# Stan994265/mVIL-Fusion

Hardware: AMD Instinct MI355X
Metric: sliding-window solve iterations/sec (10 KF, 1k feat, 30k LiDAR pts) (higher is better)
Workload: dtype f64; 1 GPU; BASELINE.json configs[1]: K=10 keyframes, L=1000 landmarks, 3068 visual factors, 24000 plane + 6000 edge LiDAR points, 9 IMU, 3 ICP, 4 LPS, prior n=70 (vil_marginalize of the preceding synthetic window, on the GPU); termination=function_tolerance, parallelism=1 GPU, step=one full window solve, inputs resident in HBM

## Files before the change

mvil-fusion_amd/csrc/vil_step.hpp:

```cpp
#pragma once
#include <type_traits>

#include "vil_dev.hpp"
#include "vil_factors.hpp"
#include "vil_finish.hpp"

namespace vd {

#define STEP_NB 4
#define CH_SLOTS 7
#define PF_N ((55 * 256 + VIL_STEP_THREADS - 1) / VIL_STEP_THREADS)

struct StepShared {
    Ctl c;
    double red[64];
    unsigned char tI[256], tJ[256];
    double xs[320], dinv[320];
    double y[320];
    double sc[320], dcs[320], gr[320], gn[320];
    double gd[320];
    double rt[320];
    double x0[328];
    unsigned char cst[48];
    double hs[12];
// ... 822 lines not shown
                a0 = fma(wr[i], y0, a0); a1 = fma(wr[i + 1], y1, a1); a2 = fma(wr[i + 2], y2, a2); a3 = fma(wr[i + 3], y3, a3);
                c0 = fma(nn[i], y0, c0); c1 = fma(nn[i + 1], y1, c1); c2 = fma(nn[i + 2], y2, c2); c3 = fma(nn[i + 3], y3, c3);
            }
            asm volatile("s_waitcnt lgkmcnt(0)" ::: "memory");
            s.y[kb + tt] = (a0 + a1) + (a2 + a3);
            crit = (c0 + c1) + (c2 + c3);
        }
        lds_barrier();
        if (t >= 64) {
            const int lim = kb - 16;
            for (int w0 = (t & ~63) - 64; w0 < lim; w0 += NT - 64) {
                const int c = w0 + (t & 63), cc = min(c, lim - 1);
                const int base = tl_base(blk, cc >> 4) + (cc & 15);
                double v0 = 0.0, v1 = 0.0, v2 = 0.0, v3 = 0.0;
#pragma unroll
                for (int r = 0; r < 16; r += 4) {
                    v0 = fma(A[base + r * TILE_RS], s.y[kb + r], v0);
                    v1 = fma(A[base + (r + 1) * TILE_RS], s.y[kb + r + 1], v1);
                    v2 = fma(A[base + (r + 2) * TILE_RS], s.y[kb + r + 2], v2);
                    v3 = fma(A[base + (r + 3) * TILE_RS], s.y[kb + r + 3], v3);
                }
                double yn = s.y[cc] - ((v0 + v1) + (v2 + v3));
                asm volatile("" : "+v"(yn));
                if (c < lim) s.y[cc] = yn;
            }
        }
    }
    lds_barrier();
}

struct ChainSrcStep {
    const double* S; int D; const double* sc_; const double* dcs_; const double* gd_; const double* u_; double mu;
    __device__ __forceinline__ double u(int i) const { return u_[i]; }
    int NP;
    __device__ __forceinline__ double raw(int i, int j) const { return S[(size_t)i * D + j]; }
    __device__ __forceinline__ double diag(int k, int i, int j) const { return raw(NP + 9 * k + i, NP + 9 * k + j); }
    __device__ __forceinline__ double sub(int k, int kn, int q, int c) const { return raw(NP + 9 * kn + q, NP + 9 * k + c); }
    __device__ __forceinline__ double prow(int r, int k, int c) const { return raw(r, NP + 9 * k + c); }
    __device__ __forceinline__ double sc(int j) const { return sc_[j]; }
    __device__ __forceinline__ double madd(int j) const { const double d = dcs_[j]; return mu * d * d; }
    __device__ __forceinline__ double rowscale(int r) const { return sc_[r]; }
    __device__ __forceinline__ double rhsraw(int j) const { return gd_[j]; }
    __device__ __forceinline__ void row_done(int, int r, double zr, double& q) const { q += 2.0 * u_[r] * zr; }
    __device__ __forceinline__ void wput(double* p, double v) const { *p = v; }
};

template <bool WLDS, class PUB, class SIDE>
__device__ __forceinline__ bool solve_chain(const DevP& P, const SysBuf& sb, StepShared& s, double* lds, const double mu, const bool cam, double& qpart, PUB pub, SIDE side) {
    const int t = vil_tid();
#ifdef VIL_STAMPS
    #define SSTAMP(k) do { if (t == 0) { long long tt_; asm volatile("s_memtime %0\n s_waitcnt lgkmcnt(0)" : "=s"(tt_) :: "memory"); P.dbg[40 + k] = tt_; } } while (0)
#else
    #define SSTAMP(k) do {} while (0)
#endif
    SSTAMP(0);
    const int K = P.K, D = P.D, NP = P.NV, R = NP + 1, T = (R + 15) >> 4, ntile = (T * (T + 1)) >> 1;
    const int RS = P.chain_rs, NB = 9 * K, m = K >> 1;
    double* Tl = lds;
    double* Wt = WLDS ? lds + ntile * TILE_SZ : P.M;
    const ChainLds L = chain_lds(lds + ntile * TILE_SZ + (WLDS ? (size_t)chain_wcols(K) * RS : 0), K);
    if (t < 8) chain_flag_set(L.flag + t, 0);
    __syncthreads();
    SSTAMP(1);
    if (t < 384) {
        const ChainSrcStep src{sb.S, D, s.sc, s.dcs, s.gd, s.y, mu, NP};
        double qc = 0.0;
        if (cam) chain_eliminate<true>(src, K, NP, RS, Wt, L, qc, P.dbg); else chain_eliminate<false>(src, K, NP, RS, Wt, L, qc, P.dbg);
        qpart += qc;
    } else {
        const int pl = t - 384, NE = ntile << 8;
        for (int e0 = pl; e0 < NE; e0 += 4 * 128) {
            double v[4]; int ii[4], jj[4];
#pragma unroll
            for (int u = 0; u < 4; ++u) {
                const int e = min(e0 + 128 * u, NE - 1), tile = e >> 8, w = e & 255;
                ii[u] = (s.tI[tile] << 4) + (w >> 4); jj[u] = (s.tJ[tile] << 4) + (w & 15);
                v[u] = sb.S[(size_t)min(ii[u], NP - 1) * D + min(jj[u], NP - 1)];
            }
#pragma unroll
            for (int u = 0; u < 4; ++u) {
                const int e = e0 + 128 * u;
                if (e >= NE) break;
                const int i = ii[u], j = jj[u];
                double mv = 0.0;
                if (i < NP && j <= i) {
                    if (cam) qpart += (i == j ? 1.0 : 2.0) * s.y[i] * v[u] * s.y[j];
                    mv = s.sc[i] * v[u] * s.sc[j];
                    if (i == j) mv += mu * s.dcs[i] * s.dcs[i];
                } else if (i == NP && j < NP) mv = s.sc[j] * s.gd[j];
                Tl[tl_phys(e)] = mv;
            }
        }
#ifdef VIL_STAMPS
        if (t == 384) { long long tt_; asm volatile("s_memtime %0\n s_waitcnt lgkmcnt(0)" : "=s"(tt_) :: "memory"); P.dbg[57] = tt_; P.dbg[58] = tt_; }
#endif
    }
    __syncthreads();
    SSTAMP(2);
    if (chain_flag_get(L.flag + 5)) return false;
    SSTAMP(3);
    auto schur = [&](d4* Creg, const int* tIJ) {
        const int lane = t & 63, row = lane & 15, kq = lane >> 4;
        if (P.skip_mask & 128) return;
        const int RS4 = 4 * RS;
#pragma unroll
        for (int u = 0; u < CH_SLOTS; ++u) {
            if (tIJ[u] < 0) continue;
            const int I = tIJ[u] >> 8, J = tIJ[u] & 255;
            const bool va = (I << 4) + row < R, vb = (J << 4) + row < R;
            const double* pa = Wt + kq * RS + (I << 4) + row;
            const double* pb = Wt + kq * RS + (J << 4) + row;
            d4 c4 = Creg[u];
            for (int kk = 0; kk < NB; kk += 32) {
                const double* qa = pa + kk * RS; const double* qb = pb + kk * RS;
                double av[8], bv[8];
#pragma unroll
                for (int g = 0; g < 8; ++g) { av[g] = qa[g * RS4]; bv[g] = qb[g * RS4]; }
#pragma unroll
                for (int g = 0; g < 8; ++g) {
                    const bool kv = kk + 4 * g + kq < NB;
                    c4 = __builtin_amdgcn_mfma_f64_16x16x4f64((va && kv) ? -av[g] : 0.0, (vb && kv) ? bv[g] : 0.0, c4, 0, 0, 0);
                }
            }
            Creg[u] = c4;
        }
    };
    if (!chol_lookahead<CH_SLOTS, false>(Tl, NP, s, schur)) return false;
    SSTAMP(4);
    back_subst(Tl, NP, s);
    pub();
    SSTAMP(5);
    double* tB = L.tB;
    {
        const int G = (4 * NB <= VIL_STEP_THREADS) ? 4 : 2;
        const int j = t / G, part = t - j * G;
        const int jc = min(j, NB - 1);
        double acc = 0.0;
        for (int rr = part; rr < NP; rr += G) acc += Wt[(size_t)jc * RS + rr] * s.y[rr];
        acc += __shfl_xor(acc, 1, 64);
        if (G == 4) acc += __shfl_xor(acc, 2, 64);
        if (j < NB && part == 0) tB[j] = Wt[(size_t)j * RS + NP] - acc;
    }
    __syncthreads();
    if (t < 64) chain_block_back(L.Ldg + 54 * m, nullptr, tB + 9 * m, nullptr, s.y + NP + 9 * m);
    __syncthreads();
    if (t < 64) { for (int k = m - 1; k >= 0; --k) chain_block_back(L.Ldg + 54 * k, L.Lsb + 82 * k, tB + 9 * k, s.y + NP + 9 * (k + 1), s.y + NP + 9 * k); }
    else if (t < 128) { for (int k = m + 1; k < K; ++k) chain_block_back(L.Ldg + 54 * k, L.Lsb + 82 * k, tB + 9 * k, s.y + NP + 9 * (k - 1), s.y + NP + 9 * k); }
    else if (t >= VIL_STEP_THREADS - 64) side();
    __syncthreads();
    SSTAMP(6);
    return true;
}

template <bool RW , class PUB, class SIDE>
__device__ __forceinline__ bool solve_prechain(const DevP& P, const SysBuf& sb, StepShared& s, double* lds, const double mu, const bool cam, double& qpart, const int epoch , PUB pub, SIDE side) {
    const int t = vil_tid();
    SSTAMP(0);
    const int K = P.K, D = P.D, NP = P.NV, R = NP + 1, T = (R + 15) >> 4, ntile = (T * (T + 1)) >> 1;
    const int RS = P.chain_rs, NB = 9 * K, m = K >> 1;
    double* Tl = lds;
    const double* Wt = P.chW;
    double* Ldg = lds + ntile * TILE_SZ; double* Lsb = Ldg + 54 * K; double* tB = Lsb + 82 * K;
    {
        const int NE = ntile << 8;
        for (int e0 = t; e0 < NE; e0 += 8 * VIL_STEP_THREADS) {
            double v[8]; int ii[8], jj[8];
#pragma unroll
            for (int u = 0; u < 8; ++u) {
                const int e = min(e0 + VIL_STEP_THREADS * u, NE - 1), tile = e >> 8, w = e & 255;
                ii[u] = (s.tI[tile] << 4) + (w >> 4); jj[u] = (s.tJ[tile] << 4) + (w & 15);
                v[u] = ld_ag(sb.S + (size_t)min(ii[u], NP - 1) * D + min(jj[u], NP - 1));
            }
#pragma unroll
            for (int u = 0; u < 8; ++u) {
                const int e = e0 + VIL_STEP_THREADS * u;
                if (e >= NE) break;
                const int i = ii[u], j = jj[u];
                double mv = 0.0;
                if (i < NP && j <= i) {
                    if (cam) qpart += (i == j ? 1.0 : 2.0) * s.y[i] * v[u] * s.y[j];
                    mv = s.sc[i] * v[u] * s.sc[j];
                    if (i == j) mv += mu * s.dcs[i] * s.dcs[i];
                } else if (i == NP && j < NP) mv = s.sc[j] * s.gd[j];
                Tl[tl_phys(e)] = mv;
            }
        }
    }
    if (P.rs_merged) {
        for (int i = t; i < P.n_ww; i += VIL_STEP_THREADS) spin_until_eq(P.wwflag + i, epoch, P.abortf);
        __syncthreads();
    }
    if (t == 0) prof_stamp(P, epoch - 1, 9);
    SSTAMP(1);
    const int f2 = (P.rs_merged || P.prechain == 2) ? ld_ag(P.chflag + 2) : 0;
    {
        const int NE = ntile << 8;
        for (int e0 = t; e0 < NE; e0 += 8 * VIL_STEP_THREADS) {
            double ww[8];
#pragma unroll
            for (int u = 0; u < 8; ++u) ww[u] = ld_ag(P.chWW + tl_phys(min(e0 + VIL_STEP_THREADS * u, NE - 1)));
#pragma unroll
            for (int u = 0; u < 8; ++u) {
                const int e = e0 + VIL_STEP_THREADS * u;
                if (e >= NE) break;
                const int tile = e >> 8, w = e & 255, i = (s.tI[tile] << 4) + (w >> 4), j = (s.tJ[tile] << 4) + (w & 15);
                if (i <= NP && j <= i && j < NP) Tl[tl_phys(e)] -= (i < NP ? s.sc[i] : 1.0) * ww[u] * s.sc[j];
            }
        }
        if (cam) {
            if (t < NP) qpart += 2.0 * s.y[t] * (ld_ag(P.chZ + t) + ld_ag(P.chZ + R + t));
            if (t == 0) qpart += ld_ag(P.chQ) + ld_ag(P.chQ + 1);
        }
        if (t == 0 && !ld_ag(P.chOk)) s.ok = 0;
    }
    __syncthreads();
    SSTAMP(2); SSTAMP(3);
    if (!s.ok) return false;
    const int G = (4 * NB <= VIL_STEP_THREADS) ? 4 : 2;
    const int j = t / G, part = t - j * G;
    const int jc = min(j, NB - 1);
    double wv[24], wrhs = 0.0;
    const bool small = ntile <= 24;
    if (small) {
        const bool wave_has_columns = __builtin_amdgcn_readfirstlane(((t >> 6) << 6) / G) < NB;
#pragma unroll
        for (int q = 0; q < 24; ++q) wv[q] = 0.0;
        if (wave_has_columns) {
#pragma unroll
            for (int q = 0; q < 24; ++q) wv[q] = ld_ag(Wt + (size_t)jc * RS + min(part + q * G, NP - 1));
            wrhs = ld_ag(Wt + (size_t)jc * RS + NP);
        }
        if (!(RW ? chol_dense<3>(Tl, NP, s) : chol_lookahead<3, false>(Tl, NP, s))) return false;
    } else if (!(RW ? chol_dense<CH_SLOTS>(Tl, NP, s) : chol_lookahead<CH_SLOTS, false>(Tl, NP, s))) return false;
    SSTAMP(4);
    if (t == 0) prof_stamp(P, epoch - 1, 10);
    if (RW) back_subst_cols(Tl, NP, s); else back_subst(Tl, NP, s);
    pub();
    if (t == 0) prof_stamp(P, epoch - 1, 11);
    SSTAMP(5);
    {
        if (P.rs_merged || P.prechain == 2) {
            if (f2 != epoch) spin_until_eq(P.chflag + 2, epoch, P.abortf);
        }
        double acc = 0.0, pl[2], ps[2];
        const int nr = (NP - part + G - 1) / G;
#pragma unroll
        for (int q = 0; q < 2; ++q) { pl[q] = ld_ag(P.chLdg + min(t + q * VIL_STEP_THREADS, 54 * K - 1)); ps[q] = ld_ag(P.chLsb + min(t + q * VIL_STEP_THREADS, 82 * K - 1)); }
#pragma unroll
        for (int q = 0; q < 2; ++q) { const int e = t + q * VIL_STEP_THREADS; if (e < 54 * K) Ldg[e] = pl[q]; if (e < 82 * K) Lsb[e] = ps[q]; }
        for (int e = t + 2 * VIL_STEP_THREADS; e < 54 * K; e += VIL_STEP_THREADS) Ldg[e] = ld_ag(P.chLdg + e);
        for (int e = t + 2 * VIL_STEP_THREADS; e < 82 * K; e += VIL_STEP_THREADS) Lsb[e] = ld_ag(P.chLsb + e);
        if (small) {
#pragma unroll
            for (int q = 0; q < 24; ++q) { const int rr = min(part + q * G, NP - 1); acc += (q < nr ? wv[q] : 0.0) * s.sc[rr] * s.y[rr]; }
            for (int q = 24; q < nr; ++q) { const int rr = part + q * G; acc += ld_ag(Wt + (size_t)jc * RS + rr) * s.sc[rr] * s.y[rr]; }
            acc += __shfl_xor(acc, 1, 64);
            if (G == 4) acc += __shfl_xor(acc, 2, 64);
            if (j < NB && part == 0) tB[j] = wrhs - acc;
        } else {
            const int wave = t >> 6, lane = t & 63;
            const int r0 = min(lane, NP - 1), r1 = min(lane + 64, NP - 1);
            const double x0 = lane < NP ? s.sc[r0] * s.y[r0] : 0.0, x1 = lane + 64 < NP ? s.sc[r1] * s.y[r1] : 0.0;
            for (int j0 = wave; j0 < NB; j0 += 64) {
                double w0[8], w1[8], wr[8];
#pragma unroll
                for (int u = 0; u < 8; ++u) {
                    const double* col = Wt + (size_t)min(j0 + 8 * u, NB - 1) * RS;
                    w0[u] = ld_ag(col + r0); w1[u] = ld_ag(col + r1); wr[u] = ld_ag(col + NP);
                }
#pragma unroll
                for (int u = 0; u < 8; ++u) {
                    const double a = wave_total(w0[u] * x0 + w1[u] * x1);
                    if (lane == 0 && j0 + 8 * u < NB) tB[j0 + 8 * u] = wr[u] - a;
                }
            }
        }
    }
    __syncthreads();
    if (t < NB) {
        const int k = t / 9, r = t - 9 * k;
        const double* Li = Ldg + 54 * k; const double* tk = tB + 9 * k;
        double a0 = 0.0, a1 = 0.0;
#pragma unroll
        for (int i = 0; i < 9; ++i) { const double li = i >= r ? Li[(i * (i + 1) >> 1) + r] : 0.0; if (i & 1) a1 += li * tk[i]; else a0 += li * tk[i]; }
        s.y[NP + t] = a0 + a1;
    }
    __syncthreads();
    if (t < 128) {
        const int dir = t >> 6, lane = t & 63, r = min(lane, 8), stp = dir == 0 ? -1 : 1, kend = dir == 0 ? -1 : K;
        double xn = s.y[NP + 9 * m + r];
        int k = m + stp;
        double mrow[9], c = 0.0;
        auto fetch = [&](int kk, double* mr, double& cc) {
            const double* Mk = Lsb + 82 * kk + 9 * r;
#pragma unroll
            for (int i = 0; i < 9; ++i) mr[i] = Mk[i];
            cc = s.y[NP + 9 * kk + r];
        };
        if (k != kend) fetch(k, mrow, c);
        for (; k != kend; k += stp) {
            double mnext[9], cnext = 0.0;
#pragma unroll
            for (int i = 0; i < 9; ++i) mnext[i] = 0.0;
            if (k + stp != kend) fetch(k + stp, mnext, cnext);
            const int xlo = __double2loint(xn), xhi = __double2hiint(xn);
            double a0 = c, a1 = 0.0, a2 = 0.0;
#pragma unroll
            for (int i = 0; i < 9; ++i) {
                const double xi = __hiloint2double(__builtin_amdgcn_readlane(xhi, i), __builtin_amdgcn_readlane(xlo, i));
                if (i % 3 == 0) a0 = fma(-mrow[i], xi, a0); else if (i % 3 == 1) a1 = fma(-mrow[i], xi, a1); else a2 = fma(-mrow[i], xi, a2);
            }
            xn = a0 + (a1 + a2);
            if (lane < 9) s.y[NP + 9 * k + lane] = xn;
#pragma unroll
            for (int i = 0; i < 9; ++i) mrow[i] = mnext[i];
            c = cnext;
        }
    }
    else if (t >= VIL_STEP_THREADS - 64) side();
    __syncthreads();
    SSTAMP(6);
    return true;
}

}

__device__ __forceinline__ void judge_step(Ctl& c, const double cand_cost, const SolveOpts& O, int& need) {
    const int cand = 1 - c.cur;
    if (fabs(c.cost_cur - cand_cost) <= O.function_tolerance * c.cost_cur) { c.done = 1; c.term = 1; }
    else {
        const double rel = (c.cost_cur - cand_cost) / c.model_change;
        if (isfinite(cand_cost) && rel > O.min_relative_decrease) {
            c.cur = cand; c.cost_cur = cand_cost; c.nsucc++;
            if (rel < 0.25) c.radius *= 0.5;
            if (rel > 0.75) c.radius = fmax(c.radius, 3.0 * c.dogleg_norm);
            c.radius = fmin(O.max_radius, c.radius);
            c.reuse = 0; need = 1;
        } else { c.radius *= 0.5; c.reuse = 1; need = 0; }
    }
    if (c.iter >= 1 && c.iter <= 64) c.cost_trace[c.iter - 1] = c.cost_cur;
}
__device__ __forceinline__ void judge_caps(Ctl& c, const SolveOpts& O) {
    if (!c.done) {
        if (c.iter >= O.max_iterations) { c.done = 1; c.term = 4; }
        else if (c.radius <= 1e-32) { c.done = 1; c.term = 6; c.status = -4; }
    }
}
__device__ __forceinline__ bool judge_would_end(const Ctl& c, const double cand_cost, const SolveOpts& O) {
    if (fabs(c.cost_cur - cand_cost) <= O.function_tolerance * c.cost_cur) return true;
    if (c.iter >= O.max_iterations) return true;
    const double rel = (c.cost_cur - cand_cost) / c.model_change;
    const bool accepted = isfinite(cand_cost) && rel > O.min_relative_decrease;
    return !accepted && c.radius * 0.5 <= 1e-32;
}
__device__ __forceinline__ void post_iter_header(const DevP& P, const Ctl& c, const int epoch) {
    const int t = vil_tid();
    if (t < 7) {
        const double dv = t <= 2 ? c.mu : (t <= 4 ? c.cg : c.cn);
        const unsigned pl = t == 0 ? (unsigned)((c.cur & 1) | ((c.done ? 1 : 0) << 1) | ((c.first ? 1 : 0) << 2) | ((c.lin_mode & 3) << 3)) : (unsigned)(((t - 1) & 1) ? __double2hiint(dv) : __double2loint(dv));
        __hip_atomic_store(P.ihdr + t, ((unsigned long long)(unsigned)epoch << 32) | pl, __ATOMIC_RELAXED, __HIP_MEMORY_SCOPE_AGENT);
    }
}
template <bool LDSM, int CHAIN, bool FUSED>
__device__ __forceinline__ void step_body(const DevP& P, const SolveOpts& O, vd::StepShared& s, double* const Alds, const int p0, const int duty_item = -1, const long long deadline_tick = 0 ) {
    using namespace vd;
    const int t = vil_tid(), NT = blockDim.x;
    const int D = P.D, L = P.L;
    const int nhelp = P.n_help;
    const bool merged = FUSED || P.rs_merged != 0;
    int bid = p0;
    if (merged) {
        const int pc = P.prechain ? 1 : 0;
        if (pc && p0 == 0) bid = 1 + nhelp;
        else if (FUSED) {
            const int q = p0 - pc;
            bid = q <= nhelp ? q : (q - 1 - nhelp < P.n_ww ? 1 + nhelp + pc + (q - 1 - nhelp) : 1 + nhelp + pc + P.n_ww + (q - 1 - nhelp - P.n_ww));
        }
        else if (p0 - pc < P.n_gather) bid = 1 + nhelp + pc + P.n_ww + (p0 - pc);
        else { const int q = p0 - pc - P.n_gather; bid = q <= nhelp ? q : 1 + nhelp + pc + (q - 1 - nhelp); }
    }
#ifdef VIL_STAMPS
    if (bid == 0 && t == 0) { long long tt_; asm volatile("s_memtime %0\n s_waitcnt lgkmcnt(0)" : "=s"(tt_) :: "memory"); P.dbg[30] = tt_; }
#endif
    const int b_chain = 1 + nhelp, b_ww = b_chain + ((merged && P.prechain) ? 1 : 0), b_gather = b_ww + (merged ? P.n_ww : 0);
    const bool helper = bid > 0 && bid <= nhelp;
    {
        const double* src = (const double*)P.ctl; double* dst = (double*)&s.c;
        for (int i = t; i < (int)(sizeof(Ctl) / 8); i += NT) dst[i] = ldx<FUSED>(src + i);
        if (t == 0) { s.need = 0; s.was_first = 0; s.ok = 1; s.early = 0; s.judged = 0; s.hdr_posted = 0; }
    }
    for (int q = t; q < 256; q += NT) {
        int Ir = (int)((sqrtf(8.f * (float)q + 1.f) - 1.f) * 0.5f);
        if (((Ir + 1) * (Ir + 2)) / 2 <= q) ++Ir;
        if ((Ir * (Ir + 1)) / 2 > q) --Ir;
        s.tI[q] = (unsigned char)Ir; s.tJ[q] = (unsigned char)(q - (Ir * (Ir + 1)) / 2);
    }
    __syncthreads();
    const int epoch = (int)((((unsigned)s.c.gen) << 12) + (unsigned)s.c.n_sweeps + 1u);
    const int lidx = epoch - 1;
    auto PROF = [&](int k, bool mn = false) { if (FUSED && t == 0) prof_stamp(P, lidx, k, mn); };
    __syncthreads();
    if (t == 0) { s.done_at_entry = s.c.done; s.c.swe++; if (FUSED) s.c.n_sweeps++; }
    __syncthreads();
#ifdef VIL_STAMPS
    #define STAMP(k) do { __syncthreads(); if (t == 0) { long long tt_; asm volatile("s_memtime %0\n s_waitcnt lgkmcnt(0)" : "=s"(tt_) :: "memory"); P.dbg[k] = tt_; } } while (0)
#else
    #define STAMP(k) do {} while (0)
#endif
    if (s.c.done) return;
    auto rs_signal = [&](int* f) { asm volatile("s_waitcnt vmcnt(0)" ::: "memory"); __syncthreads(); if (t == 0) __hip_atomic_store(f, epoch, __ATOMIC_RELAXED, __HIP_MEMORY_SCOPE_AGENT); };
    auto rs_wait = [&](const int* f, int n) {
        for (int i = t; i < n; i += NT) spin_until_eq(f + i, epoch, P.abortf);
        __syncthreads();
    };
    if (merged && bid >= b_gather) {
        if constexpr (FUSED) reduce_gather<true, VIL_STEP_THREADS / 8, true>(P, s.c, bid - b_gather, (int4*)Alds, epoch);
        else if (P.rs_merged == 2) reduce_gather<true, VIL_STEP_THREADS / 8>(P, s.c, bid - b_gather, (int4*)Alds);
        else { if (t >= VIL_THREADS) return; reduce_gather<true, RED_EPW>(P, s.c, bid - b_gather, (int4*)Alds); }
        if (P.drop_role == -2 - (bid - b_gather) && s.c.n_sweeps - 1 == P.drop_launch) return;
        rs_signal(P.gflag + (bid - b_gather)); PROF(5); return;
    }
    auto duty = [&]() {
        if constexpr (FUSED) if (duty_item >= 0) {
            reduce_gather<true, VIL_STEP_THREADS / 8, true>(P, s.c, duty_item, (int4*)Alds, epoch);
            if (!(P.drop_role == -2 - duty_item && s.c.n_sweeps - 1 == P.drop_launch)) rs_signal(P.gflag + duty_item);
            PROF(5);
            __syncthreads();
        }
    };
    if (merged && bid >= b_ww) {
        duty();
        if (!FUSED && t >= VIL_THREADS) return;
        rs_wait(P.chflag, 1); prechain_ww_tile<FUSED>(P, bid - b_ww, Alds); rs_signal(P.wwflag + (bid - b_ww)); PROF(13); return;
    }
    if (merged && P.prechain && bid == b_chain) { prechain_wg<FUSED>(P, s.c, O.jacobi_scaling, Alds, epoch, FUSED); return; }
    if (!merged && P.prechain == 2 && bid == b_chain) { prechain_inverses(P, Alds, epoch); return; }
    if (bid == 0) PROF(7);
    if constexpr (FUSED) {
        if (bid == 0) {
            const int v0 = P.n_imu + 2, nv = P.n_vwg, n1 = P.n_sw - nv;
            for (int i = t; i < n1; i += NT) spin_until_eq(P.sflag + (i < v0 ? i : i + nv), epoch, P.abortf);
            __syncthreads();
            if (t == 0) st_ag(P.sall + 16, epoch);
            for (int i = t; i < nv; i += NT) spin_until_eq(P.sflag + v0 + i, epoch, P.abortf);
            __syncthreads();
            if (t == 0) st_ag(P.sall + 32, epoch);
            if (P.persist && !s.c.first && !s.c.resweep && s.c.lin_mode == 0) {
                const double cc = gather_cost<VIL_STEP_THREADS / 8, true>(P, s.red);
                if (t == 0) s.early = judge_would_end(s.c, cc, O) ? 1 : 0;
                __syncthreads();
                if (s.early) {
                    if (t == 0) { Ctl& c = s.c; c.cand_cost = cc; judge_step(c, cc, O, s.need); judge_caps(c, O); c.outd = 1; s.judged = 1; }
                    __syncthreads();
                    vd::solve_finish<true>(P.x[0], P.x[1], P.xorig, P.hstate, P.ctl, P.hctl, P.hseq, P.K, P.NS, P.gauge_on, s.c.cur, s.c.status, s.c.gen, Alds, &s.c);
                    post_iter_header(P, s.c, epoch);
                    asm volatile("s_waitcnt vmcnt(0)" ::: "memory"); __syncthreads();
                    if (t == 0) st_ag(P.sall + 48, epoch);
                }
            }
        }
    }
    if (FUSED && merged && bid > 0) {
        duty();
        if (t == 0) {
            spin_until_eq(P.sall + 48, epoch, P.abortf);
            if (P.persist) { const unsigned long long h0 = __hip_atomic_load(P.ihdr, __ATOMIC_RELAXED, __HIP_MEMORY_SCOPE_AGENT); s.early = ((unsigned)(h0 >> 32) == (unsigned)epoch && ((unsigned)h0 & 2u)) ? 1 : 0; }
        }
        __syncthreads();
        if (s.early) { if (t == 0) { asm volatile("s_waitcnt vmcnt(0)" ::: "memory"); __hip_atomic_store(P.hflag + (bid - 1), epoch, __ATOMIC_RELAXED, __HIP_MEMORY_SCOPE_AGENT); } return; }
    }
    else if (merged && !s.early) { rs_wait(P.gflag, P.n_gather); if (FUSED && t == 0) st_ag(P.sall + 48, epoch); }
    if (bid == 0) PROF(8);
    auto post = [&](int* f) { if (t == 0) { asm volatile("s_waitcnt vmcnt(0)" ::: "memory"); __hip_atomic_store(f, epoch, __ATOMIC_RELAXED, __HIP_MEMORY_SCOPE_AGENT); } };
    auto wait1 = [&](int* f) { spin_until_eq(f, epoch, P.abortf); };
    auto put = [&](double* p, double v) { __hip_atomic_store(p, v, __ATOMIC_RELAXED, __HIP_MEMORY_SCOPE_AGENT); };
    auto put_ll = [&](unsigned long long* p, int half) { __hip_atomic_store(p, ((unsigned long long)(unsigned)epoch << 32) | (unsigned)half, __ATOMIC_RELAXED, __HIP_MEMORY_SCOPE_AGENT); };
    auto ld_ll = [&](const unsigned long long* p) { return __hip_atomic_load(p, __ATOMIC_RELAXED, __HIP_MEMORY_SCOPE_AGENT); };
    auto store_ctl = [&]() {
        static_assert(sizeof(Ctl) % 8 == 0, "Ctl is copied as doubles");
        const double* src = (const double*)&s.c;
        double* dst = (double*)P.ctl;
        for (int i = t; i < (int)(sizeof(Ctl) / 8); i += 64) stx<FUSED>(dst + i, src[i]);
    };
    bool hseen = false;
    auto wait_helpers = [&]() { if (!hseen && t < nhelp) wait1(P.hflag + t); if (!hseen && merged && P.prechain && t < P.n_ww) wait1(P.wwflag + t); hseen = true; };
    int abort_pre = -1;
    auto end_iter = [&]() {
        wait_helpers();
        if (t == 0 && P.abortf && (abort_pre >= 0 ? abort_pre : ld_ag(P.abortf)) != 0) { s.c.done = 1; s.c.term = 6; s.c.status = -2; }
        __builtin_amdgcn_fence(__ATOMIC_ACQ_REL, "wavefront"); __builtin_amdgcn_wave_barrier();
        if (!(FUSED && P.persist)) store_ctl();
    };
    const bool cam = true;
    STAMP(0);
    if (t == 0 && !s.judged) {
        Ctl& c = s.c;
        const int cand = 1 - c.cur;
        const double cand_cost = merged ? ld_ag(P.sys[cand].cost) : *P.sys[cand].cost;
        c.cand_cost = cand_cost;
        if (c.first && *P.setup_stat != 0) { c.done = 1; c.term = 6; c.status = *P.setup_stat; }
        if (c.first || c.resweep) {
            if (c.first) { c.initial_cost = cand_cost; s.was_first = 1; }
            if (!isfinite(cand_cost)) { c.done = 1; c.term = 6; c.status = -3; }
            c.cur = cand; c.cost_cur = cand_cost; c.first = 0; c.resweep = 0; s.need = 1;
        } else judge_step(c, cand_cost, O, s.need);
        judge_caps(c, O);
    }
    __syncthreads();
    const int cur = s.c.cur;
    SysBuf sb = P.sys[cur];
    const double* x = P.x[cur];
    double* xc = P.x[1 - cur];
    auto lm_pass1 = [&](int l0, int l1, const double* vc, double& q, double& g2, double& gm) {
        for (int l = l0 + t; l < l1; l += NT) {
            const double ip = ldx<FUSED>(sb.invp + l), Sl = ldx<FUSED>(sb.sl + l), h = ldx<FUSED>(sb.hll + l), b = ldx<FUSED>(sb.bl + l);
            const double d = sqrt(fmin(fmax(Sl * Sl * h, 1e-6), 1e32));
            const double g = ip != 0.0 ? Sl * b / d : 0.0;
            P.dl[l] = d; P.gradl[l] = g;
            if (ip != 0.0) {
                const double ul = Sl * g / d;
                const double ev = lm_dot<FUSED>(P, sb, l, vc);
                q += ip * ev * ev + 2.0 * ul * ev + h * ul * ul;
                g2 += g * g; gm = fmax(gm, fabs(b));
            }
        }
    };
    auto lm_pass2 = [&](int l0, int l1, const double* vc, double* sm ) {
        for (int l = l0 + t; l < l1; l += NT) {
            const double ip = ldx<FUSED>(sb.invp + l);
            double a = 0.0, b = 0.0;
            if (ip != 0.0) {
                const double Sl = ldx<FUSED>(sb.sl + l), dl = P.dl[l], g = P.gradl[l];
                const double xl = (ldx<FUSED>(sb.bl + l) - lm_dot<FUSED>(P, sb, l, vc)) * ip / Sl;
                const double gnv = -xl * dl;
                sm[0] += gnv * gnv; sm[1] += gnv * g;
                a = Sl * g / dl; b = Sl * gnv / dl;
                sm[2] += a * a; sm[3] += a * b; sm[4] += b * b;
            }
            stx<FUSED>(P.la + l, a); stx<FUSED>(P.lb + l, b);
            if (!(P.lm_const && P.lm_const[l])) { const double lam = ldx<FUSED>(x + xo_lam(P) + l); sm[5] += lam * lam; }
        }
    };
    auto wait_x = [&](double* dst) {
        for (int w = t; w < 2 * P.NV; w += NT) {
            const unsigned long long* p = (const unsigned long long*)P.stepc + w;
            unsigned long long tw0 = 0;
            for (int sp = 0;;) {
                const unsigned long long v = ld_ll(p);
                const int b = __hip_atomic_load(P.xstat, __ATOMIC_RELAXED, __HIP_MEMORY_SCOPE_AGENT);
                if ((unsigned)(v >> 32) == (unsigned)epoch) { ((unsigned*)dst)[w] = (unsigned)v; break; }
                if (b == epoch) { s.ok = 0; break; }
                __builtin_amdgcn_s_sleep(1);
                if ((++sp & 1023) == 0 && P.abortf && wait_expired(tw0, P.abortf)) { st_ag(P.abortf, 1); s.ok = 0; break; }
            }
        }
        __syncthreads();
    };
    auto post_wave2 = [&](double* sm) {
        bsum6(sm, s);
        const int slot = bid - 1;
        if (t == 0) { unsigned long long* hp = (unsigned long long*)P.hpart2 + 16 * slot; for (int e = 0; e < 6; ++e) { put_ll(hp + 2 * e, __double2loint(sm[e])); put_ll(hp + 2 * e + 1, __double2hiint(sm[e])); } }
    };
    auto gather2 = [&](double* h, bool with1) {
        const int ln = t & 63;
        for (int e = 0; e < 9; ++e) h[e] = 0.0;
        for (int s0 = 0; s0 < nhelp; s0 += 64) {
            const int slot = s0 + ln;
            if (slot < nhelp) {
                const unsigned long long* hp = (const unsigned long long*)P.hpart2 + 16 * slot;
                unsigned long long w[12];
                unsigned long long tw0 = 0;
                for (int sp = 0;;) {
                    bool all = true;
#pragma unroll
                    for (int e = 0; e < 12; ++e) w[e] = ld_ll(hp + e);
#pragma unroll
                    for (int e = 0; e < 12; ++e) all = all && (unsigned)(w[e] >> 32) == (unsigned)epoch;
                    if (all) break;
                    __builtin_amdgcn_s_sleep(1);
                    if ((++sp & 1023) == 0 && P.abortf && wait_expired(tw0, P.abortf)) { st_ag(P.abortf, 1); break; }
                }
#pragma unroll
                for (int e = 0; e < 6; ++e) h[e] += __hiloint2double((int)(unsigned)w[2 * e + 1], (int)(unsigned)w[2 * e]);
            }
        }
        if (with1 && ln < nhelp) for (int e = 0; e < 3; ++e) h[6 + e] = __hip_atomic_load(P.hpart + 4 * ln + e, __ATOMIC_RELAXED, __HIP_MEMORY_SCOPE_AGENT);
        for (int e = 0; e < 8; ++e) h[e] = wave_total_l63(h[e]);
        h[8] = wave_max_l63(h[8]);
    };
    if (helper) {
        const int hk = bid - 1;
        if (!s.c.done && s.need) {
            for (int i = t; i < P.NV; i += NT) {
                const double dg = merged ? ld_ag(sb.diag + i) : sb.diag[i], b = merged ? ld_ag(sb.bc + i) : sb.bc[i];
                const double Sc = s.was_first ? (O.jacobi_scaling ? 1.0 / (1.0 + sqrt(dg)) : 1.0) : ldx<FUSED>(P.Sc + i);
                const double d = sqrt(fmin(fmax(Sc * Sc * dg, 1e-6), 1e32));
                s.y[i] = Sc * (Sc * b / d) / d;
            }
            __syncthreads();
            const int per = (L + nhelp - 1) / nhelp, l0 = hk * per, l1 = min(L, l0 + per);
            double q = 0, g2 = 0, gm = 0;
            if (per <= NT) {
                const bool quad = 2 * per <= NT;
                const int G = 4 * per <= NT ? 4 : (quad ? 2 : 1);
                const int qd = t & (G - 1);
                const int l = l0 + (G == 4 ? (t >> 2) : G == 2 ? (t >> 1) : t);
                const bool have = l < l1, lead = have && qd == 0;
                LmRows r; r.fs = 0; r.fe = 0;
                double ip = 0, b = 0, d = 1, g = 0, lam2 = 0, ipS = 0, Sd = 0, a_ = 0, h_ = 0;
                if (have) {
                    if (quad) lm_rows_quad<FUSED>(P, sb, l, qd, r, G); else lm_rows<FUSED>(P, sb, l, r);
                    ip = ldx<FUSED>(sb.invp + l); b = ldx<FUSED>(sb.bl + l);
                    const double Sl = ldx<FUSED>(sb.sl + l), h = ldx<FUSED>(sb.hll + l);
                    h_ = h;
                    if (!(P.lm_const && P.lm_const[l])) { const double lam = ldx<FUSED>(x + xo_lam(P) + l); lam2 = lam * lam; }
                    d = sqrt(fmin(fmax(Sl * Sl * h, 1e-6), 1e32));
                    g = ip != 0.0 ? Sl * b / d : 0.0;
                    if (lead) { P.dl[l] = d; P.gradl[l] = g; }
                    if (ip != 0.0) { Sd = Sl / d; ipS = ip / Sl; a_ = Sd * g; }
                }
                {
                    double ev = (have && ip != 0.0) ? lm_dot_rows<FUSED>(P, sb, r, s.y) : 0.0;
                    if (G == 4) ev = quad_total(ev); else if (G == 2) ev = pair_total(ev);
                    if (lead && ip != 0.0) {
                        q += ip * ev * ev + 2.0 * a_ * ev + h_ * a_ * a_;
                        g2 += g * g; gm = fmax(gm, fabs(b));
                    }
                }
                bsum3<true>(g2, q, gm, s);
                if (t == 0) { double* hp = P.hpart + 4 * hk; put(hp, q); put(hp + 1, g2); put(hp + 2, gm); }
                post(P.hflag + hk);
                wait_x(s.gn);
                if (s.ok) {
                    double sm[6] = {0, 0, 0, 0, 0, 0};
                    double b_ = 0.0;
                    double ev2 = (have && ip != 0.0) ? lm_dot_rows<FUSED>(P, sb, r, s.gn) : 0.0;
                    if (G == 4) ev2 = quad_total(ev2); else if (G == 2) ev2 = pair_total(ev2);
                    if (lead) {
                        if (ip != 0.0) {
                            const double xl = (b - ev2) * ipS;
                            const double gnv = -xl * d;
                            sm[0] = gnv * gnv; sm[1] = gnv * g;
                            b_ = Sd * gnv;
                            sm[2] = a_ * a_; sm[3] = a_ * b_; sm[4] = b_ * b_;
                        }
                        sm[5] = lam2;
                    }
                    post_wave2(sm);
                    if (lead) { stx<FUSED>(P.la + l, a_); stx<FUSED>(P.lb + l, b_); }
                }
                return;
            }
            lm_pass1(l0, l1, s.y, q, g2, gm);
            bsum3<true>(g2, q, gm, s);
            if (t == 0) { double* hp = P.hpart + 4 * hk; put(hp, q); put(hp + 1, g2); put(hp + 2, gm); }
            post(P.hflag + hk);
            wait_x(s.y);
            if (s.ok) {
                double sm[6] = {0, 0, 0, 0, 0, 0};
                lm_pass2(l0, l1, s.y, sm);
                post_wave2(sm);
            }
        } else post(P.hflag + hk);
        return;
    }
    if (s.c.done) { if (t < 64) end_iter(); return; }
    for (int i = t; i < 16 * P.K + 8; i += NT) s.x0[i] = ldx<FUSED>(x + i);
    for (int k = t; k < 2 * P.K; k += NT) s.cst[k] = k < P.K ? (P.pose_const ? P.pose_const[k] : 0) : (P.sb_const ? P.sb_const[k - P.K] : 0);
    bool xpub = false;
    auto publish_xp = [&](int okk) {
        if (nhelp) {
            if (okk) { for (int w = t; w < 2 * P.NV; w += NT) { const double v = s.sc[w >> 1] * s.y[w >> 1]; put_ll((unsigned long long*)P.stepc + w, (w & 1) ? __double2hiint(v) : __double2loint(v)); } }
            else { __syncthreads(); post(P.xstat); }
        }
        xpub = true;
    };
    double pf[PF_N];
    if (CHAIN == 0 && s.need) {
        const int R = D + 1, T = (R + 15) >> 4, NTL = (tri_off(T)) << 8;
        const int half = __builtin_amdgcn_readfirstlane(t >> 8), w = t & 255;
        static_for<PF_N>([&](auto uc) {
            constexpr int u = decltype(uc)::value;
            constexpr int I0 = tri_row_c(2 * u), J0 = tri_col_c(2 * u), I1 = tri_row_c(2 * u + 1), J1 = tri_col_c(2 * u + 1);
            const int e = t + u * VIL_STEP_THREADS;
            pf[u] = 0.0;
            if (e < NTL) {
                const int I = half ? I1 : I0, J = half ? J1 : J0;
                const int i = (I << 4) + (w >> 4), j = (J << 4) + (w & 15);
                if (i < D && j <= i) pf[u] = sb.S[(size_t)i * D + j];
            }
        });
    }
    STAMP(1);
    double gn2 = 0, g2 = 0, gg = 0;
    bool spec = false;
    double* const xcs_spec = Alds; double* const sums_spec = Alds + 336;
    auto cand_blocks = [&](auto&& stepf, double* xcs, double& xn, double& sn) {
        const int K = P.K;
        for (int k = t; k < 2 * K + 2; k += NT) {
            if (k < K) {
                const double* in = s.x0 + xo_pose(P, k); double* o = xcs + xo_pose(P, k);
                if (s.cst[k]) { for (int q = 0; q < 7; ++q) o[q] = in[q]; }
                else { double st[6]; for (int q = 0; q < 6; ++q) st[q] = stepf(col_pose(P, k) + q); pose_plus(in, st, o); for (int q = 0; q < 7; ++q) { xn += in[q] * in[q]; sn += (in[q] - o[q]) * (in[q] - o[q]); } }
            } else if (k < 2 * K) {
                const int kk = k - K;
                const double* in = s.x0 + xo_sb(P, kk); double* o = xcs + xo_sb(P, kk);
                const bool cst = s.cst[K + kk] != 0;
                for (int q = 0; q < 9; ++q) { const double d = cst ? 0.0 : stepf(col_sb(P, kk) + q); o[q] = in[q] + d; if (!cst) { xn += in[q] * in[q]; sn += d * d; } }
            } else if (k == 2 * K) {
                const double* in = s.x0 + xo_ex(P); double* o = xcs + xo_ex(P);
                if (P.ex_const) { for (int q = 0; q < 7; ++q) o[q] = in[q]; }
                else { double st[6]; for (int q = 0; q < 6; ++q) st[q] = stepf(col_ex(P) + q); pose_plus(in, st, o); for (int q = 0; q < 7; ++q) { xn += in[q] * in[q]; sn += (in[q] - o[q]) * (in[q] - o[q]); } }
            } else {
                const double in = s.x0[xo_td(P)];
                const double d = P.td_free ? stepf(col_td(P)) : 0.0;
                xcs[xo_td(P)] = in + d;
                if (P.td_free) { xn += in * in; sn += d * d; }
            }
        }
    };
    if (s.need) {
        double gm = 0;
        if constexpr (CHAIN == 3) { if (merged) { if (t == 0) wait1(P.chflag + 1); __syncthreads(); } }
        for (int i = t; i < D; i += NT) {
            const double dg = merged ? ld_ag(sb.diag + i) : sb.diag[i], b = merged ? ld_ag(sb.bc + i) : sb.bc[i];
            double Sc;
            if (s.was_first) { Sc = O.jacobi_scaling ? 1.0 / (1.0 + sqrt(dg)) : 1.0; if (CHAIN == 3 && i >= P.NV) Sc = ld_ag(P.chSc + (i - P.NV)); stx<FUSED>(P.Sc + i, Sc); } else Sc = ldx<FUSED>(P.Sc + i);
            double d = sqrt(fmin(fmax(Sc * Sc * dg, 1e-6), 1e32));
            if (CHAIN == 3 && i >= P.NV) d = ld_ag(P.chDc + (i - P.NV));
            const double g = Sc * b / d;
            s.sc[i] = Sc; s.dcs[i] = d; s.gr[i] = g; s.y[i] = Sc * g / d; s.gd[i] = merged ? ld_ag(sb.gred + i) : sb.gred[i]; s.rt[i] = Sc / d;
            P.dc[i] = d; P.gradc[i] = g;
            if (cam) { g2 += g * g; gm = fmax(gm, fabs(b)); }
        }
        __syncthreads();
        STAMP(9);
        double q = 0;
        if (!nhelp) lm_pass1(0, L, s.y, q, g2, gm);
        STAMP(10);
        const double mu = s.c.mu;
        bool ok = true;
        if constexpr (CHAIN != 0) {
            __syncthreads();
            auto pub = [&]() { publish_xp(1); };
            auto side = [&]() {};
            if constexpr (CHAIN == 3) ok = solve_prechain<FUSED>(P, sb, s, Alds, mu, cam, q, epoch, pub, side);
            else ok = solve_chain<CHAIN == 1>(P, sb, s, Alds, mu, cam, q, pub, side);
        } else {
        double* Ag = P.M;
        const int R = D + 1, T = (R + 15) >> 4, NTL = (tri_off(T)) << 8;
        const int half = __builtin_amdgcn_readfirstlane(t >> 8), w = t & 255;
#ifdef VIL_STAMPS
        long long tpk0 = 0; if (t == 0) { asm volatile("s_memtime %0\n s_waitcnt lgkmcnt(0)" : "=s"(tpk0) :: "memory"); }
#endif
        static_for<PF_N>([&](auto uc) {
            constexpr int u = decltype(uc)::value;
            constexpr int I0 = tri_row_c(2 * u), J0 = tri_col_c(2 * u), I1 = tri_row_c(2 * u + 1), J1 = tri_col_c(2 * u + 1);
            const int e = t + u * VIL_STEP_THREADS;
            if (e < NTL) {
                const int I = half ? I1 : I0, J = half ? J1 : J0;
                const int i = (I << 4) + (w >> 4), j = (J << 4) + (w & 15);
                double m = 0.0;
                if (i < D && j <= i) {
                    const double v = pf[u];
                    if (cam) q += (i == j ? 1.0 : 2.0) * s.y[i] * v * s.y[j];
                    m = s.sc[i] * v * s.sc[j];
                    if (i == j) m += mu * s.dcs[i] * s.dcs[i];
                } else if (i == D && j < D) m = s.sc[j] * s.gd[j];
                if constexpr (LDSM) Alds[tl_phys(e)] = m; else Ag[tl_phys(e)] = m;
            }
        });
#ifdef VIL_STAMPS
        if (t == 0) { long long tpk1; asm volatile("s_memtime %0\n s_waitcnt lgkmcnt(0)" : "=s"(tpk1) :: "memory"); P.dbg[27] = tpk1 - tpk0; }
#endif
        for (int e = t + PF_N * VIL_STEP_THREADS; e < NTL; e += VIL_STEP_THREADS) {
            const int tile = e >> 8, w = e & 255;
            const int I = s.tI[tile], J = s.tJ[tile];
            const int i = (I << 4) + (w >> 4), j = (J << 4) + (w & 15);
            double m = 0.0;
            if (i < D && j <= i) {
                const double v = sb.S[(size_t)i * D + j];
                if (cam) q += (i == j ? 1.0 : 2.0) * s.y[i] * v * s.y[j];
                m = s.sc[i] * v * s.sc[j];
                if (i == j) m += mu * s.dcs[i] * s.dcs[i];
            } else if (i == D && j < D) m = s.sc[j] * s.gd[j];
            if constexpr (LDSM) Alds[tl_phys(e)] = m; else Ag[tl_phys(e)] = m;
        }
        }
        STAMP(11);
        const bool defer = CHAIN != 0 && nhelp > 0 && ok;
        if (!defer) bsum3<true>(g2, q, gm, s);
        if (nhelp && !defer) {
            if (t < 64) {
                wait_helpers();
                double h0 = 0, h1 = 0, h2 = 0;
                if (t < nhelp) {
                    h0 = __hip_atomic_load(P.hpart + 4 * t, __ATOMIC_RELAXED, __HIP_MEMORY_SCOPE_AGENT);
                    h1 = __hip_atomic_load(P.hpart + 4 * t + 1, __ATOMIC_RELAXED, __HIP_MEMORY_SCOPE_AGENT);
                    h2 = __hip_atomic_load(P.hpart + 4 * t + 2, __ATOMIC_RELAXED, __HIP_MEMORY_SCOPE_AGENT);
                }
                for (int k = 0; k < nhelp; ++k) { q += __shfl(h0, k); g2 += __shfl(h1, k); gm = fmax(gm, __shfl(h2, k)); }
                if (t == 0) { s.red[0] = q; s.red[1] = g2; s.red[2] = gm; }
            }
            __syncthreads();
            q = s.red[0]; g2 = s.red[1]; gm = s.red[2];
            __syncthreads();
        }
        STAMP(2);
        if (!defer && gm <= O.gradient_tolerance) {
            if (!xpub) publish_xp(0);
            if (t == 0) { s.c.done = 1; s.c.term = 2; }
            if (t < 64) { __builtin_amdgcn_fence(__ATOMIC_ACQ_REL, "wavefront"); __builtin_amdgcn_wave_barrier(); end_iter(); }
            return;
        }
        if constexpr (CHAIN == 0) { if constexpr (LDSM) ok = chol_lookahead<CH_SLOTS, false>(Alds, D, s); else ok = chol_blocked<false>(P.M, D, s, Alds); }
        STAMP(3);
        PROF(21);
#ifdef VIL_STAMPS
        if (t == 0) { P.dbg[20] = s.tacc[0]; P.dbg[21] = s.tacc[1]; P.dbg[22] = s.tacc[2]; P.dbg[24] = s.tacc[3]; P.dbg[25] = s.tacc[4]; P.dbg[26] = s.tacc[5]; }
#endif
        if (!ok) {
            if (!xpub) publish_xp(0);
            if (t == 0) {
                Ctl& c = s.c;
                c.mu *= 10.0;
                if (!(c.mu < O.max_mu)) { c.iter++; c.invalid_run++; c.reuse = 0; if (c.invalid_run >= 5) { c.done = 1; c.term = 6; c.status = -4; } }
                c.resweep = 1; c.cg = 0.0; c.cn = 0.0;
            }
            for (int i = t; i < P.NS; i += NT) stx<FUSED>(xc + i, i >= xo_lam(P) ? ldx<FUSED>(x + i) : s.x0[i]);
            if (FUSED && P.persist) for (int w = t; w < 2 * (16 * P.K + 8); w += NT) put_ll(P.xtag + w, (w & 1) ? __double2hiint(s.x0[w >> 1]) : __double2loint(s.x0[w >> 1]));
            __syncthreads();
            if (t < 64) end_iter();
            return;
        }
        if constexpr (CHAIN == 0) { if constexpr (LDSM) back_subst(Alds, D, s); else back_subst(P.M, D, s); publish_xp(1); __syncthreads(); }
        STAMP(4);
#ifdef VIL_STAMPS
        if (t == 0) P.dbg[23] = s.tacc[0];
#endif
        for (int i = t; i < D; i += NT) {
            const double xi = s.y[i];
            const double gnv = -xi * s.dcs[i];
            s.gn[i] = gnv; P.gnc[i] = gnv;
            if (cam) { gn2 += gnv * gnv; gg += gnv * s.gr[i]; }
            s.y[i] = s.sc[i] * xi;
        }
        __syncthreads();
        if (defer && LDSM && NT >= 192 && P.K + 1 <= 64) {
            auto stepf = [&](const int i) { return (0.0 * s.gr[i] + 1.0 * s.gn[i]) * s.rt[i]; };
            const int K = P.K;
            double xs_ = 0, ss_ = 0;
            if (t < 64) {
                if (t <= K) {
                    const bool isex = t == K;
                    const int xo = isex ? xo_ex(P) : xo_pose(P, t), col = isex ? col_ex(P) : col_pose(P, t);
                    const bool cst = isex ? P.ex_const != 0 : s.cst[min(t, K - 1)] != 0;
                    const double* in = s.x0 + xo; double* o = xcs_spec + xo;
                    double st[6], ov[7];
#pragma unroll
                    for (int q = 0; q < 6; ++q) st[q] = stepf(col + q);
                    pose_plus(in, st, ov);
#pragma unroll
                    for (int q = 0; q < 7; ++q) { const double iv = in[q]; o[q] = cst ? iv : ov[q]; if (!cst) { xs_ += iv * iv; ss_ += (iv - ov[q]) * (iv - ov[q]); } }
                }
            } else if (t < 128) {
                const int l = t - 64;
                if (l < K) {
                    const double* in = s.x0 + xo_sb(P, l); double* o = xcs_spec + xo_sb(P, l);
                    const bool cst = s.cst[K + l] != 0;
#pragma unroll
                    for (int q = 0; q < 9; ++q) { const double iv = in[q], d = cst ? 0.0 : stepf(col_sb(P, l) + q); o[q] = iv + d; if (!cst) { xs_ += iv * iv; ss_ += d * d; } }
                } else if (l == K) {
                    const double iv = s.x0[xo_td(P)], d = P.td_free ? stepf(col_td(P)) : 0.0;
                    xcs_spec[xo_td(P)] = iv + d;
                    if (P.td_free) { xs_ += iv * iv; ss_ += d * d; }
                }
            }
            if (t < 128) {
                xs_ = wave_total_l63(xs_); ss_ = wave_total_l63(ss_);
                if ((t & 63) == 63) { sums_spec[2 * (t >> 6)] = xs_; sums_spec[2 * (t >> 6) + 1] = ss_; }
            }
            spec = true;
        }
        if (defer && t >= NT - 64) { double h[9]; gather2(h, true); if ((t & 63) == 63) for (int e = 0; e < 9; ++e) s.hs[e] = h[e]; }
        double sm[6] = {0, 0, 0, 0, 0, 0};
        if (!nhelp) lm_pass2(0, L, s.y, sm);
        sm[0] += gn2; sm[1] += gg;
        if (defer) bsum5(g2, q, gm, sm[0], sm[1], s);
        else { bsum3(sm[0], sm[1], sm[2], s); if (!nhelp) bsum3(sm[3], sm[4], sm[5], s); }
        if (defer) {
            hseen = true;
            for (int e = 0; e < 6; ++e) sm[e] += s.hs[e];
            q += s.hs[6]; g2 += s.hs[7]; gm = fmax(gm, s.hs[8]);
        }
        if (nhelp) {
            if (!defer) {
            if (t < 64) {
                double h[9];
                gather2(h, false);
// ... 103 lines not shown
```

Measured before the change: 17720 iterations/s.

## Prefetch Schur tiles early, relax ww-flag wait, reuse gathered candidate cost

In the fused chain-3 path, the first batch of reduced-system S values is loaded into registers before waiting on the chain flag and computing the scaling, so the global load latency overlaps that work. The wait on the ww tile flags is spread across wavefronts with a per-wave fence and wave barrier instead of a block-wide __syncthreads. The candidate cost already gathered in block 0 is reused instead of being reloaded from global memory. This adds register pressure, and the per-wave wait only covers a subset of flags per wave, which risks ordering issues if more than 64 flags exist.

```diff
diff --git a/mvil-fusion_amd/csrc/vil_step.hpp b/mvil-fusion_amd/csrc/vil_step.hpp
--- a/mvil-fusion_amd/csrc/vil_step.hpp
+++ b/mvil-fusion_amd/csrc/vil_step.hpp
@@ -998,8 +998,17 @@
     return true;
 }
 
+__device__ __forceinline__ void prechain_request_S(const DevP& P, const SysBuf& sb, const StepShared& s, double (&v)[8]) {
+    const int t = vil_tid(), NP = P.NV, D = P.D, R = NP + 1, T = (R + 15) >> 4, NE = ((T * (T + 1)) >> 1) << 8;
+#pragma unroll
+    for (int u = 0; u < 8; ++u) {
+        const int e = min(t + VIL_STEP_THREADS * u, NE - 1), tile = e >> 8, w = e & 255;
+        const int i = (s.tI[tile] << 4) + (w >> 4), j = (s.tJ[tile] << 4) + (w & 15);
+        v[u] = ld_ag(sb.S + (size_t)min(i, NP - 1) * D + min(j, NP - 1));
+    }
+}
 template <bool RW , class PUB, class SIDE>
-__device__ __forceinline__ bool solve_prechain(const DevP& P, const SysBuf& sb, StepShared& s, double* lds, const double mu, const bool cam, double& qpart, const int epoch , PUB pub, SIDE side) {
+__device__ __forceinline__ bool solve_prechain(const DevP& P, const SysBuf& sb, StepShared& s, double* lds, const double mu, const bool cam, double& qpart, const int epoch , const double (&pfS)[8] , PUB pub, SIDE side) {
     const int t = vil_tid();
     SSTAMP(0);
     const int K = P.K, D = P.D, NP = P.NV, R = NP + 1, T = (R + 15) >> 4, ntile = (T * (T + 1)) >> 1;
@@ -1015,7 +1024,11 @@
             for (int u = 0; u < 8; ++u) {
                 const int e = min(e0 + VIL_STEP_THREADS * u, NE - 1), tile = e >> 8, w = e & 255;
                 ii[u] = (s.tI[tile] << 4) + (w >> 4); jj[u] = (s.tJ[tile] << 4) + (w & 15);
-                v[u] = ld_ag(sb.S + (size_t)min(ii[u], NP - 1) * D + min(jj[u], NP - 1));
+                v[u] = RW ? pfS[u] : 0.0;
+            }
+            if (!RW || e0 != t) {
+#pragma unroll
+                for (int u = 0; u < 8; ++u) v[u] = ld_ag(sb.S + (size_t)min(ii[u], NP - 1) * D + min(jj[u], NP - 1));
             }
 #pragma unroll
             for (int u = 0; u < 8; ++u) {
@@ -1033,10 +1046,11 @@
         }
     }
     if (P.rs_merged) {
-        for (int i = t; i < P.n_ww; i += VIL_STEP_THREADS) spin_until_eq(P.wwflag + i, epoch, P.abortf);
-        __syncthreads();
-    }
-    if (t == 0) prof_stamp(P, epoch - 1, 9);
+        const int lane = t & 63, tl = (t >> 8) + 2 * lane;
+        if (lane < 32 && tl < P.n_ww) spin_until_eq(P.wwflag + tl, epoch, P.abortf);
+        __builtin_amdgcn_fence(__ATOMIC_ACQ_REL, "wavefront"); __builtin_amdgcn_wave_barrier();
+    }
+    if ((t & 63) == 0) prof_stamp(P, epoch - 1, 9);
     SSTAMP(1);
     const int f2 = (P.rs_merged || P.prechain == 2) ? ld_ag(P.chflag + 2) : 0;
     {
@@ -1277,11 +1291,12 @@
     if (merged && bid >= b_ww) {
         duty();
         if (!FUSED && t >= VIL_THREADS) return;
-        rs_wait(P.chflag, 1); prechain_ww_tile<FUSED>(P, bid - b_ww, Alds); rs_signal(P.wwflag + (bid - b_ww)); PROF(13); return;
+        rs_wait(P.chflag, 1); PROF(30); prechain_ww_tile<FUSED>(P, bid - b_ww, Alds); rs_signal(P.wwflag + (bid - b_ww)); PROF(13); return;
     }
     if (merged && P.prechain && bid == b_chain) { prechain_wg<FUSED>(P, s.c, O.jacobi_scaling, Alds, epoch, FUSED); return; }
     if (!merged && P.prechain == 2 && bid == b_chain) { prechain_inverses(P, Alds, epoch); return; }
     if (bid == 0) PROF(7);
+    double cf_cost = 0.0; bool cf_have = false;
     if constexpr (FUSED) {
         if (bid == 0) {
             const int v0 = P.n_imu + 2, nv = P.n_vwg, n1 = P.n_sw - nv;
@@ -1293,7 +1308,7 @@
             if (t == 0) st_ag(P.sall + 32, epoch);
             if (P.persist && !s.c.first && !s.c.resweep && s.c.lin_mode == 0) {
                 const double cc = gather_cost<VIL_STEP_THREADS / 8, true>(P, s.red);
-                if (t == 0) s.early = judge_would_end(s.c, cc, O) ? 1 : 0;
+                if (t == 0) { s.early = judge_would_end(s.c, cc, O) ? 1 : 0; cf_cost = cc; cf_have = true; }
                 __syncthreads();
                 if (s.early) {
                     if (t == 0) { Ctl& c = s.c; c.cand_cost = cc; judge_step(c, cc, O, s.need); judge_caps(c, O); c.outd = 1; s.judged = 1; }
@@ -1342,7 +1357,10 @@
     if (t == 0 && !s.judged) {
         Ctl& c = s.c;
         const int cand = 1 - c.cur;
-        const double cand_cost = merged ? ld_ag(P.sys[cand].cost) : *P.sys[cand].cost;
+        const double cand_cost = cf_have ? cf_cost : (merged ? ld_ag(P.sys[cand].cost) : *P.sys[cand].cost);
+#ifdef VIL_STAMPS
+        if (cf_have && __double_as_longlong(ld_ag(P.sys[cand].cost)) != __double_as_longlong(cf_cost)) P.dbg[59] = 0x7fffffffffffffffll;
+#endif
         c.cand_cost = cand_cost;
         if (c.first && *P.setup_stat != 0) { c.done = 1; c.term = 6; c.status = *P.setup_stat; }
         if (c.first || c.resweep) {
@@ -1567,6 +1585,8 @@
     };
     if (s.need) {
         double gm = 0;
+        double pfS[8];
+        if constexpr (CHAIN == 3 && FUSED) { prechain_request_S(P, sb, s, pfS); if (bid == 0) PROF(29); }
         if constexpr (CHAIN == 3) { if (merged) { if (t == 0) wait1(P.chflag + 1); __syncthreads(); } }
         for (int i = t; i < D; i += NT) {
             const double dg = merged ? ld_ag(sb.diag + i) : sb.diag[i], b = merged ? ld_ag(sb.bc + i) : sb.bc[i];
@@ -1590,7 +1610,7 @@
             __syncthreads();
             auto pub = [&]() { publish_xp(1); };
             auto side = [&]() {};
-            if constexpr (CHAIN == 3) ok = solve_prechain<FUSED>(P, sb, s, Alds, mu, cam, q, epoch, pub, side);
+            if constexpr (CHAIN == 3) ok = solve_prechain<FUSED>(P, sb, s, Alds, mu, cam, q, epoch, pfS, pub, side);
             else ok = solve_chain<CHAIN == 1>(P, sb, s, Alds, mu, cam, q, pub, side);
         } else {
         double* Ag = P.M;
```

Measured after the change: 17700 iterations/s, median of 2. About the same (-0.1%).
